# NoemieJaquier/GaBOtorch

Hardware: AMD Instinct MI355X
Metric: SPD affine-invariant kernel-matrix build, pairs/sec (N=4096,d=10) (higher is better)
Workload: dtype f64

## Files before the change

### gabotorch_amd/csrc/spd_pairwise_body.hpp

```cpp
#pragma once
#include "gabo_device.hpp"
#include "spd_eig.hpp"
#include "spd_prep.hpp"
#include "gabo_mirror.hpp"
#include "spd_generic.hpp"
#include "gabo_log_tab.hpp"
#include "gabo_exp_tab256.hpp"
#include "gabo_acosh2_table.hpp"
#include "../../include/gabo_hip.h"

#ifndef GABO_PAIR_WAVES
#define GABO_PAIR_WAVES 2
#else
#define GABO_PAIR_WAVES_FORCED 1
#endif

namespace gabo {

typedef const double __attribute__((address_space(1)))* spd_gcol_ptr;

struct SpdGcolBuffer {
    __amdgpu_buffer_rsrc_t rsrc;
    int voff;
    int stride_bytes;
    __device__ __forceinline__ double operator[](int k) const {
        return __builtin_bit_cast(double, __builtin_amdgcn_raw_buffer_load_b64(rsrc, voff, k * stride_bytes, 0));
    }
};
struct SpdGcolPointer {
    spd_gcol_ptr p;
    int64_t stride;
    __device__ __forceinline__ double operator[](int k) const { return p[(int64_t)k * stride]; }
};

template <int D, int WLIM>
struct SpdWGroups {
    int n = 0;
    int col[tri_size(D)] = {}, r0[tri_size(D)] = {}, r1[tri_size(D)] = {};
    constexpr SpdWGroups() {
        static_assert(WLIM >= D, "a row of the first column must fit a group");
        for (int c = D - 1; c >= 0; --c) {
            for (int r = c; r < D;) {
                int sum = 0;
                col[n] = c, r0[n] = r;
                while (r < D && sum + (r - c + 1) <= WLIM) sum += r - c + 1, ++r;
                r1[n++] = r;
            }
        }
    }
};
#ifndef GABO_PAIR_WLIM
#define GABO_PAIR_WLIM 16
#endif
template <int D, int AHEAD, class GCOL>
__device__ __forceinline__ void ai_congruence_staged(const double* __restrict__ W, const GCOL& Gj, double (&m)[tri_size(D)]) {
    constexpr SpdWGroups<D, (GABO_PAIR_WLIM < D ? D : GABO_PAIR_WLIM)> kG{};
    double gq[D][D];
    double wq[2][D][D];
    double c[D];
    auto issue_g = [&](auto ss) {
        constexpr int col = D - 1 - decltype(ss)::value;
        static_for<D - col>([&](auto kk) { gq[col][decltype(kk)::value] = Gj[tri(col + decltype(kk)::value, col)]; });
    };
    auto issue_w = [&](auto gg) {
        constexpr int g = decltype(gg)::value, col = kG.col[g], r0 = kG.r0[g], r1 = kG.r1[g];
        typedef const double __attribute__((address_space(4)))* wrow_ptr;
        wrow_ptr Wg = (wrow_ptr)W;
        asm volatile("" : "+s"(Wg));
        static_for<r1 - r0>([&](auto rr) {
            constexpr int r = r0 + decltype(rr)::value;
            static_for<r - col + 1>([&](auto kk) { wq[g & 1][r][col + decltype(kk)::value] = Wg[tri(r, col + decltype(kk)::value)]; });
        });
    };
    static_for<(AHEAD < D ? AHEAD : D)>(issue_g);
    issue_w(std::integral_constant<int, 0>{});
    static_for<kG.n>([&](auto gg) {
        constexpr int g = decltype(gg)::value, col = kG.col[g], r0 = kG.r0[g], r1 = kG.r1[g];
        if constexpr (r0 == col && D - 1 - col + AHEAD < D) issue_g(std::integral_constant<int, D - 1 - col + AHEAD>{});
        __builtin_amdgcn_sched_barrier(0);
        __builtin_amdgcn_s_waitcnt(0xc07f);
        __builtin_amdgcn_sched_barrier(0);
        if constexpr (g + 1 < kG.n) issue_w(std::integral_constant<int, g + 1>{});
        static_for<r1 - r0>([&](auto rr) {
            constexpr int r = r0 + decltype(rr)::value;
            double acc = wq[g & 1][r][col] * gq[col][0];
            static_for<r - col>([&](auto kk) {
                constexpr int k = col + 1 + decltype(kk)::value;
                acc = __builtin_fma(wq[g & 1][r][k], gq[col][k - col], acc);
            });
            c[r - col] = acc;
        });
        if constexpr (r1 == D) {
            __builtin_amdgcn_sched_barrier(0);
            static_for<D - col>([&](auto rr) {
                constexpr int r = col + decltype(rr)::value;
                static_for<r - col + 1>([&](auto qq) {
                    constexpr int q = col + decltype(qq)::value;
                    m[tri(r, q)] = col == q ? c[r - col] * c[q - col] : __builtin_fma(c[r - col], c[q - col], m[tri(r, q)]);
                });
            });
        }
    });
    __builtin_amdgcn_sched_barrier(0);
}

__constant__ double kLogTabRegs[8] = {1.41421356237309504880, 1.0 / 7.0, -1.0 / 6.0, 0.2, -0.25, 1.0 / 3.0, 6.93147180369123816490e-01,
                                      1.90821492927058770002e-10};
__device__ __forceinline__ LogTabRegs log_tab_regs_scalar() {
    typedef const double __attribute__((address_space(4)))* const_ptr;
    const_ptr p = (const_ptr)kLogTabRegs;
    asm volatile("" : "+s"(p));
    LogTabRegs t;
    t.sqrt2 = p[0], t.c7 = p[1], t.c6 = p[2], t.c5 = p[3], t.c4 = p[4], t.c3 = p[5], t.ln2_hi = p[6], t.ln2_lo = p[7];
    return t;
}

template <int D, int ORIENT = kQlOrientPerLane, int CTL = kQlCtlPlain, int AHEAD = 0, class GCOL>
__device__ __forceinline__ double ai_sumsq(const double* __restrict__ W, const GCOL& Gj, const double* __restrict__ ltab, const double eps2 = 0.0) {
    constexpr int T = tri_size(D);
    constexpr bool kDescending = ORIENT == kQlOrientLast;
    double m[T];
    if constexpr (AHEAD > 0) {
        static_assert(kDescending, "the staged congruence takes the columns from the last to the first");
        ai_congruence_staged<D, AHEAD>(W, Gj, m);
    } else
    static_for<D>([&](auto cc) {
        constexpr int col = kDescending ? D - 1 - decltype(cc)::value : decltype(cc)::value;
        double g[D - col], c[D - col];
        static_for<D - col>([&](auto kk) { g[decltype(kk)::value] = Gj[tri(col + decltype(kk)::value, col)]; });
        static_for<D - col>([&](auto rr) {
            constexpr int r = col + decltype(rr)::value;
            double acc = W[tri(r, col)] * g[0];
            static_for<r - col>([&](auto kk) {
                constexpr int k = col + 1 + decltype(kk)::value;
                acc = __builtin_fma(W[tri(r, k)], g[k - col], acc);
            });
            c[r - col] = acc;
        });
        static_for<D - col>([&](auto rr) {
            constexpr int r = col + decltype(rr)::value;
            static_for<r - col + 1>([&](auto qq) {
                constexpr int q = col + decltype(qq)::value;
                m[tri(r, q)] = (kDescending ? col == q : col == 0) ? c[r - col] * c[q - col] : __builtin_fma(c[r - col], c[q - col], m[tri(r, q)]);
            });
        });
    });
    double dg[D], e2[D];
    tridiagonalize<D, ORIENT>(m, dg, e2);
    tridiag_eigenvalues<D, ORIENT, CTL>(dg, e2, eps2);
    double s = 0.0;
    const LogTabRegs lr = AHEAD > 0 ? log_tab_regs_scalar() : LogTabRegs::load();
    static_for<D>([&](auto kk) { double lg = log_tab(dg[decltype(kk)::value], lr, ltab); s = __builtin_fma(lg, lg, s); });
    return s;
}

struct Spd2Col {
    double g00, g10, g11, lg;
};
__device__ __forceinline__ double ai_sumsq2(const double* __restrict__ W, const Spd2Col& g, double lw, const LogTabRegs& lr,
                                            const double* __restrict__ ltab, double tiny) {
    const double c00 = W[0] * g.g00, c11 = W[2] * g.g11;
    const double c10 = __builtin_fma(W[1], g.g00, W[2] * g.g10);
    const double m00 = c00 * c00, m10d = (c10 + c10) * c00, m11 = __builtin_fma(c10, c10, c11 * c11);
    const double tr = m00 + m11, df = m00 - m11;
    const double root = sqrt_nz(__builtin_fma(df, df, __builtin_fma(m10d, m10d, tiny)));
    const double l1 = log_tab(0.5 * (tr + root), lr, ltab);
    const double l2 = __builtin_fma(2.0, lw + g.lg, -l1);
    return __builtin_fma(l1, l1, l2 * l2);
}

__device__ __forceinline__ double finish(double dist, double beta, int mode) {
    if (mode == GABO_OUT_DISTANCE) return dist;
    if (mode == GABO_OUT_LAPLACE) return exp(-(dist * beta));
    return exp(-((dist * dist) * beta));
}

#ifndef GABO_PAIR_TWO_WAVE_MAX_DIM
#define GABO_PAIR_TWO_WAVE_MAX_DIM 14
#endif
#ifndef GABO_QL_EPS2_GAUSS
#define GABO_QL_EPS2_GAUSS 1e-14
#endif
constexpr bool spd_pair_gauss_only_instantiated(int d) { return d > 2 && d != 12; }
#ifndef GABO_PAIR_ORIENT
constexpr int spd_pair_gauss_only_orientation(int d) { return d == 14 ? kQlOrientCol0 : kQlOrientLast; }
#else
constexpr int spd_pair_gauss_only_orientation(int d) { return GABO_PAIR_ORIENT; }
#endif
#ifndef GABO_PAIR_SWEEPCTL
constexpr int spd_pair_gauss_only_sweepctl(int d) { return d == 20 ? kQlCtlPlain : (kQlCtlDenormalZero | kQlCtlHwSqrt | kQlCtlStageThreshold); }
#else
constexpr int spd_pair_gauss_only_sweepctl(int d) { return GABO_PAIR_SWEEPCTL; }
#endif
#ifndef GABO_PAIR_WAVES_FORCED
constexpr int spd_pair_gauss_only_waves(int d) { return d > GABO_PAIR_TWO_WAVE_MAX_DIM ? 1 : (d == 10 ? 3 : GABO_PAIR_WAVES); }
#else
constexpr int spd_pair_gauss_only_waves(int d) { return d > GABO_PAIR_TWO_WAVE_MAX_DIM ? 1 : GABO_PAIR_WAVES; }
#endif
#ifndef GABO_PAIR_AHEAD
constexpr int spd_pair_gauss_only_ahead(int d) { return d == 10 && spd_pair_gauss_only_waves(d) == 3 ? 2 : 0; }
#else
constexpr int spd_pair_gauss_only_ahead(int d) { return d == 10 ? GABO_PAIR_AHEAD : 0; }
#endif
template <int D, bool GAUSS_ONLY, bool BUFFER_ONLY>
__global__ __launch_bounds__(256, (GAUSS_ONLY ? spd_pair_gauss_only_waves(D) : (D > GABO_PAIR_TWO_WAVE_MAX_DIM ? 1 : GABO_PAIR_WAVES))) void spd_ai_pairwise_kernel(const double* __restrict__ Winv, const double* __restrict__ G,
                                                              double* __restrict__ out, double* __restrict__ dist_out_arg,
                                                              int64_t n1, int64_t n2,
                                                              int64_t w_batch_stride, int64_t g_batch_stride, int rows,
                                                              int col_blocks, int row_chunks, int64_t sym_tiles, double beta, int flags) {
    constexpr int T = tri_size(D);
    static_assert(GAUSS_ONLY == BUFFER_ONLY && (spd_pair_gauss_only_instantiated(D) || !GAUSS_ONLY), "instantiations that launch_spd_ai selects");
    const int mode = GAUSS_ONLY ? GABO_OUT_GAUSSIAN : (flags & GABO_OUT_MASK);
    double* const dist_out = GAUSS_ONLY ? nullptr : dist_out_arg;
    constexpr bool kTabExp = D <= 4;
    __shared__ double tab[kTabExp ? 64 : 1];
    __shared__ __attribute__((aligned(16))) double ltab[512];
    for (int k = threadIdx.x; k < 512; k += blockDim.x) ltab[k] = kLogTab[k];
    double ec[6], ec3 = 0.0;
    if constexpr (kTabExp) {
        if (threadIdx.x < 64) tab[threadIdx.x] = kExp2Tab[threadIdx.x];
    }
    __syncthreads();
    if constexpr (kTabExp) {
        static_for<6>([&](auto k) { ec[decltype(k)::value] = kExpTabC[decltype(k)::value]; });
        ec3 = ec[3];
        asm volatile("" : "+v"(ec3));
    }
    int64_t cg, rc, b;
    if (flags & GABO_SYMMETRIC) {
        const int64_t per_batch = sym_tiles;
        b = blockIdx.x / per_batch;
        int64_t t = blockIdx.x - b * per_batch;
        cg = 0;
        for (;;) {
            int64_t cnt = ((cg + 1) * (int64_t)blockDim.x + rows - 1) / rows;
            if (cnt > row_chunks) cnt = row_chunks;
            if (t < cnt) break;
            t -= cnt;
            ++cg;
        }
        rc = t;
    } else {
        const int64_t bid = blockIdx.x;
        cg = bid % col_blocks;
        rc = (bid / col_blocks) % row_chunks;
        b = bid / ((int64_t)col_blocks * row_chunks);
    }
    const int64_t j0 = cg * blockDim.x;
    const int64_t j = j0 + threadIdx.x;
    const int64_t jc = j < n2 ? j : n2 - 1;
    const int64_t i0 = rc * rows;
    const int64_t i1 = (i0 + rows < n1) ? i0 + rows : n1;
    if ((flags & GABO_SYMMETRIC) && j0 + (int64_t)(threadIdx.x | 63) < i0) return;
    const double* Gj = G + b * g_batch_stride + jc;
    double* ob = out + b * n1 * n2;
    const int64_t jw = j0 + (threadIdx.x & ~63);
    const bool use_buffer = BUFFER_ONLY || (D > 2 && (int64_t)T * n2 * 8 < (1ll << 31));
    SpdGcolBuffer gbuf;
    {
        const double* gw = G + b * g_batch_stride + (jw < n2 ? jw : n2 - 1);
        uint64_t a = (uint64_t)gw;
        a = ((uint64_t)(uint32_t)__builtin_amdgcn_readfirstlane((int)(a >> 32)) << 32) | (uint32_t)__builtin_amdgcn_readfirstlane((int)a);
        gbuf.rsrc = __builtin_amdgcn_make_buffer_rsrc((void*)a, 0, 0x7fffffff, 0x00020000);
        gbuf.voff = (int)((jc - (jw < n2 ? jw : n2 - 1)) * 8);
        gbuf.stride_bytes = (int)(n2 * 8);
    }
    Spd2Col col2;
    double lw_lane = 0.0, tiny = 1e-290;
    LogTabRegs lr2;
    if constexpr (D == 2) {
        lr2 = LogTabRegs::load();
        asm volatile("" : "+s"(tiny));
        col2.g00 = Gj[0];
        col2.g10 = Gj[n2];
        col2.g11 = Gj[2 * n2];
        col2.lg = log_tab(col2.g00 * col2.g11, lr2, ltab);
        int64_t ir = i0 + (threadIdx.x & 63);
        ir = ir < n1 ? ir : n1 - 1;
        const double* Wr = Winv + b * w_batch_stride + ir * T;
        lw_lane = log_tab(Wr[0] * Wr[2], lr2, ltab);
    }
    double eps2 = (mode == GABO_OUT_GAUSSIAN && !dist_out) ? GABO_QL_EPS2_GAUSS : 0.0;
    asm volatile("" : "+s"(eps2));
    if constexpr (GAUSS_ONLY && BUFFER_ONLY) {
        const int nrows = __builtin_amdgcn_readfirstlane((int)(i1 - i0));
        const int64_t jrel = j - i0;
        const int rmax = j >= n2 ? -1 : ((flags & GABO_SYMMETRIC) ? (jrel < 0 ? -1 : (jrel > rows - 1 ? rows - 1 : (int)jrel)) : rows - 1);
        const double* W = Winv + b * w_batch_stride + i0 * T;
        char* orow = reinterpret_cast<char*>(ob + i0 * n2 + j);
        for (int r = 0; r < nrows; ++r, W += T) {
            SpdGcolBuffer gb = gbuf;
            asm volatile("" : "+v"(gb.voff));
            asm volatile("" : "+s"(gb.stride_bytes));
            const double s = ai_sumsq<D, spd_pair_gauss_only_orientation(D), spd_pair_gauss_only_sweepctl(D), spd_pair_gauss_only_ahead(D)>(W, gb, ltab, eps2);
            double val;
            if constexpr (kTabExp) {
                val = exp_neg_tab(-((s + 1e-15) * beta), ec, ec3, tab);
                val = s != s ? s : val;
            } else {
                val = exp(-((s + 1e-15) * beta));
            }
            if (r <= rmax) *reinterpret_cast<double*>(orow) = val;
            orow += (unsigned)gb.stride_bytes;
        }
        return;
    }
    for (int64_t i = i0; i < i1; ++i) {
        const double* W = Winv + b * w_batch_stride + i * T;
        double s;
        if constexpr (D == 2) {
            const int lane = (int)(i - i0);
            const double lw = __hiloint2double(__builtin_amdgcn_readlane(__double2hiint(lw_lane), lane),
                                               __builtin_amdgcn_readlane(__double2loint(lw_lane), lane));
            s = ai_sumsq2(W, col2, lw, lr2, ltab, tiny);
        } else {
            if (use_buffer) {
                SpdGcolBuffer gb = gbuf;
                asm volatile("" : "+v"(gb.voff));
                asm volatile("" : "+s"(gb.stride_bytes));
                s = ai_sumsq<D>(W, gb, ltab, eps2);
            } else {
                SpdGcolPointer gp{(spd_gcol_ptr)Gj, n2};
                asm volatile("" : "+v"(gp.p));
                s = ai_sumsq<D>(W, gp, ltab, eps2);
            }
        }
        double dist, val;
        if (mode == GABO_OUT_GAUSSIAN && !dist_out) {
            dist = 0.0;
            if constexpr (kTabExp) {
                val = exp_neg_tab(-((s + 1e-15) * beta), ec, ec3, tab);
                val = s != s ? s : val;
            } else {
                val = exp(-((s + 1e-15) * beta));
            }
        } else {
            dist = __builtin_sqrt(s + 1e-15);
            val = finish(dist, beta, mode);
        }
        if (j < n2 && (!(flags & GABO_SYMMETRIC) || i <= j)) {
            ob[i * n2 + j] = val;
            if (dist_out) dist_out[b * n1 * n2 + i * n2 + j] = dist;
        }
    }
}

#ifndef GABO_GAUSS2_MAX_ROWS
#define GABO_GAUSS2_MAX_ROWS 64
#endif
constexpr double kGauss2L = 0.0027076061740622863;
__constant__ double kGauss2C[6] = {kGauss2L, kGauss2L * kGauss2L / 2.0, kGauss2L * kGauss2L * kGauss2L / 6.0,
                                   kGauss2L * kGauss2L * kGauss2L * kGauss2L / 24.0, 6755399441055744.0, 4096.0};

template <bool NT, bool SYM>
__global__ __launch_bounds__(256) void spd_ai_gauss2_kernel(const double* __restrict__ Winv, const double* __restrict__ G,
                                                            double* __restrict__ out, int64_t n1, int64_t n2, int64_t w_batch_stride,
                                                            int64_t g_batch_stride, int rows, int col_blocks, int row_chunks,
                                                            int64_t sym_tiles, double beta, int flags) {
    __shared__ __attribute__((aligned(16))) double ltab[512];
    __shared__ double etab[256];
    __shared__ __attribute__((aligned(16))) double atab[kAcosh2Slots * kAcosh2Stride];
    __shared__ __attribute__((aligned(16))) double wrow[GABO_GAUSS2_MAX_ROWS * 4];
    const int tid = threadIdx.x;
    for (int k = tid; k < 512; k += blockDim.x) ltab[k] = kLogTab[k];
    for (int k = tid; k < 256; k += blockDim.x) etab[k] = kExp2Tab256[k];
    {
        const double sc = beta * (-512.0 / 0.69314718055994530942), eps = beta * (-256.0 / 0.69314718055994530942) * 1e-15;
        constexpr int kUsedLo = (kAcosh2Binades - 1) * 16 * kAcosh2Stride, kUsedHi = 240 * kAcosh2Stride;
        for (int k = tid; k < kAcosh2Slots * kAcosh2Stride - (kUsedHi - kUsedLo); k += blockDim.x) {
            const int kk = k < kUsedLo ? k : k + (kUsedHi - kUsedLo);
            const double v = kAcosh2Tab[kk] * sc;
            atab[kk] = (kk % kAcosh2Stride == 0) ? v + eps : v;
        }
    }
    int64_t cg, rc, b;
    if constexpr (SYM) {
        const int64_t per_batch = sym_tiles;
        b = blockIdx.x / per_batch;
        int64_t t = blockIdx.x - b * per_batch;
        cg = 0;
        for (;;) {
            int64_t cnt = ((cg + 1) * (int64_t)blockDim.x + rows - 1) / rows;
            if (cnt > row_chunks) cnt = row_chunks;
            if (t < cnt) break;
            t -= cnt;
            ++cg;
        }
        rc = t;
    } else {
        const int64_t bid = blockIdx.x;
        cg = bid % col_blocks;
        rc = (bid / col_blocks) % row_chunks;
        b = bid / ((int64_t)col_blocks * row_chunks);
    }
    const int64_t j0 = cg * blockDim.x;
    const int64_t j = j0 + tid;
    const int64_t jc = j < n2 ? j : n2 - 1;
    const int64_t i0 = rc * rows;
    const int64_t i1 = (i0 + rows < n1) ? i0 + rows : n1;
    const double* Gj = G + b * g_batch_stride + jc;
    const double g00 = Gj[0], g10 = Gj[n2], g11 = Gj[2 * n2];
    const LogTabRegs lr = LogTabRegs::load();
    const double sscale = __builtin_sqrt(beta * (512.0 / 0.69314718055994530942));
    double w0l = 1.0, w1l = 0.0, w2l = 1.0;
    if (tid < rows) {
        int64_t ir = i0 + tid;
        ir = ir < n1 ? ir : n1 - 1;
        const double* Wr = Winv + b * w_batch_stride + ir * 3;
        w0l = Wr[0], w1l = Wr[1], w2l = Wr[2];
    }
    __syncthreads();
    if (tid < rows) {
        const double dw = w0l * w2l;
        const double sw = rsqrt_nz(dw + dw);
        wrow[4 * tid + 0] = w0l * sw;
        wrow[4 * tid + 1] = w1l * sw;
        wrow[4 * tid + 2] = w2l * sw;
        wrow[4 * tid + 3] = sscale * log_tab(dw, lr, ltab);
    }
    __syncthreads();
    if (SYM && j0 + (int64_t)(tid | 63) < i0) return;
    double ec[6];
    static_for<6>([&](auto k) { ec[decltype(k)::value] = kGauss2C[decltype(k)::value]; });
    double c4v = ec[3];
    asm volatile("" : "+v"(c4v));
    const double dg = g00 * g11;
    const double bcol = sscale * log_tab(dg, lr, ltab);
    const double sg = rsqrt_nz(dg);
    const double q00 = g00 * sg, q10 = g10 * sg, q11 = g11 * sg;
    double* orow = out + b * n1 * n2 + i0 * n2 + j;
    const int nrows = __builtin_amdgcn_readfirstlane((int)(i1 - i0));
    const int64_t jrel = j - i0;
    const int rmax = j >= n2 ? -1 : (SYM ? (jrel < 0 ? -1 : (jrel > GABO_GAUSS2_MAX_ROWS - 1 ? GABO_GAUSS2_MAX_ROWS - 1 : (int)jrel)) : GABO_GAUSS2_MAX_ROWS - 1);
    typedef double g2_v2d __attribute__((ext_vector_type(2)));
    if (!SYM && j >= n2) return;
    for (int r = 0; r < nrows; ++r, orow += n2) {
        const g2_v2d wa = *reinterpret_cast<const g2_v2d*>(wrow + 4 * r);
        const g2_v2d wb = *reinterpret_cast<const g2_v2d*>(wrow + 4 * r + 2);
        const double w0 = wa[0], w1 = wa[1], w2 = wb[0], arow = wb[1];
        const double hh = __builtin_fma(w0, q00, -(w2 * q11));
        const double cc = __builtin_fma(w1, q00, w2 * q10);
        const double tau = __builtin_fma(cc, cc, __builtin_fma(hh, hh, 1.0));
        const unsigned hi = (unsigned)__double2hiint(tau);
        static_assert(kAcosh2MBits == 4 && kAcosh2Slots == 256, "row index = 8 bits");
        const unsigned off = __umul24((hi >> 16) & 0xffu, (unsigned)(kAcosh2Stride * sizeof(double)));
        const double t = tau - __hiloint2double((int)(hi & ~((1u << (20 - kAcosh2MBits)) - 1u)), 0);
        const g2_v2d* row = reinterpret_cast<const g2_v2d*>(reinterpret_cast<const char*>(atab) + off);
        static_assert(kAcosh2Deg == 7, "four coefficient pairs");
        const g2_v2d c67 = row[3], c45 = row[2], c23 = row[1], c01 = row[0];
        double ya = __builtin_fma(c67[1], t, c67[0]);
        ya = __builtin_fma(ya, t, c45[1]);
        ya = __builtin_fma(ya, t, c45[0]);
        ya = __builtin_fma(ya, t, c23[1]);
        ya = __builtin_fma(ya, t, c23[0]);
        ya = __builtin_fma(ya, t, c01[1]);
        ya = __builtin_fma(ya, t, c01[0]);
        if (__builtin_expect(__any(!(tau < ec[5])), 0)) {
            if (!(tau < ec[5])) {
                const double dl = log(tau + __builtin_sqrt(__builtin_fma(tau, tau, -1.0)));
                ya = -(sscale * sscale) * __builtin_fma(dl, dl, 0.5e-15);
            }
        }
        const double sp = arow + bcol;
        const double y = __builtin_fma(-sp, sp, ya);
        const double km = y + ec[4];
        const double kk = km - ec[4];
        const double rr = y - kk;
        double p = __builtin_fma(rr, c4v, ec[2]);
        p = __builtin_fma(p, rr, ec[1]);
        p = __builtin_fma(p, rr, ec[0]);
        p = p * rr;
        const int ki = __double2loint(km);
        const double e = etab[ki & 255];
        const double val = __builtin_ldexp(__builtin_fma(e, p, e), ki >> 8);
        if (!SYM || r <= rmax) {
            if constexpr (NT) __builtin_nontemporal_store(val, orow);
            else *orow = val;
        }
    }
}

template <int D>
static int launch_spd_ai(const double* x1, const double* x2, double* out, double* dist_out, int64_t batch, int64_t n1, int64_t n2,
                         int64_t s1, int64_t s2, double beta, int flags, double* ws, int* status, hipStream_t st, bool prepared = false) {
    constexpr int T = tri_size(D);
    const int64_t b1 = (s1 == 0) ? 1 : batch;
    const int64_t b2 = (s2 == 0) ? 1 : batch;
    double* W = ws;
    double* G = ws + b1 * n1 * T;
    if (!prepared) launch_spd_prep<D>(x1, x2, W, G, b1, b2, n1, n2, s1, s2, status, st, 1);
#ifndef GABO_PAIR_THREADS
#define GABO_PAIR_THREADS (D >= 7 ? 64 : 256)
#endif
    int threads = n2 >= 256 ? GABO_PAIR_THREADS : (n2 > 128 ? 192 : (n2 > 64 ? 128 : 64));
    int64_t col_blocks = (n2 + threads - 1) / threads;
#ifndef GABO_PAIR_ROWS_D2
#define GABO_PAIR_ROWS_D2 16
#endif
#ifndef GABO_PAIR_ROWS
#define GABO_PAIR_ROWS (D >= 9 ? 8 : 16)
#endif
#ifndef GABO_PAIR_ROWS_GAUSS2
#define GABO_PAIR_ROWS_GAUSS2 64
#endif
    const bool gauss2 = D == 2 && (flags & GABO_OUT_MASK) == GABO_OUT_GAUSSIAN && !dist_out && beta >= 0.0;
    int rows = D == 2 ? (gauss2 ? GABO_PAIR_ROWS_GAUSS2 : GABO_PAIR_ROWS_D2) : GABO_PAIR_ROWS;
    while (rows > 1 && col_blocks * ((n1 + rows - 1) / rows) * batch < (rows > 16 ? 1024 : 4096)) rows >>= 1;
    int64_t row_chunks = (n1 + rows - 1) / rows;
    int64_t sym_tiles = 0;
    if (flags & GABO_SYMMETRIC) {
        for (int64_t cg = 0; cg < col_blocks; ++cg) {
            int64_t cnt = ((cg + 1) * threads + rows - 1) / rows;
            sym_tiles += cnt < row_chunks ? cnt : row_chunks;
        }
    }
    int64_t nblocks = ((flags & GABO_SYMMETRIC) ? sym_tiles : col_blocks * row_chunks) * batch;
    if (nblocks > 0x7fffffffLL) return GABO_ERR_ARG;
    bool special2 = false;
    if constexpr (D == 2) special2 = gauss2 && rows <= GABO_GAUSS2_MAX_ROWS;
    if (special2) {
        const bool streaming = batch * n1 * n2 * 8 > (32ll << 20) && !(flags & GABO_SYMMETRIC);
#define GABO_GAUSS2_LAUNCH(...)                                                                                                     \
        hipLaunchKernelGGL((spd_ai_gauss2_kernel<__VA_ARGS__>), dim3((unsigned)nblocks), dim3(threads), 0, st, W, G, out, n1, n2,           \
                           (s1 == 0) ? (int64_t)0 : n1 * T, (s2 == 0) ? (int64_t)0 : n2 * T, rows, (int)col_blocks, (int)row_chunks,       \
                           sym_tiles, beta, flags)
        if (flags & GABO_SYMMETRIC) GABO_GAUSS2_LAUNCH(false, true);
        else if (streaming) GABO_GAUSS2_LAUNCH(true, false);
        else GABO_GAUSS2_LAUNCH(false, false);
#undef GABO_GAUSS2_LAUNCH
    } else {
#define GABO_PAIR_LAUNCH(...)                                                                                                             \
        hipLaunchKernelGGL((spd_ai_pairwise_kernel<D, __VA_ARGS__>), dim3((unsigned)nblocks), dim3(threads), 0, st, W, G, out, dist_out, n1, n2, \
                           (s1 == 0) ? (int64_t)0 : n1 * T, (s2 == 0) ? (int64_t)0 : n2 * T, rows, (int)col_blocks, (int)row_chunks,       \
                           sym_tiles, beta, flags)
        bool gauss_only = false;
        if constexpr (spd_pair_gauss_only_instantiated(D)) {
            gauss_only = (flags & GABO_OUT_MASK) == GABO_OUT_GAUSSIAN && !dist_out && (int64_t)T * n2 * 8 < (1ll << 31);
            if (gauss_only) GABO_PAIR_LAUNCH(true, true);
        }
        if (!gauss_only) GABO_PAIR_LAUNCH(false, false);
#undef GABO_PAIR_LAUNCH
    }
    if (flags & GABO_SYMMETRIC) {
        int tiles = (int)((n1 + 31) / 32);
        hipLaunchKernelGGL((mirror_upper_kernel<0>), dim3((unsigned)((int64_t)tiles * (tiles + 1) / 2), (unsigned)batch), dim3(256), 0, st,
                           out, n1, tiles);
        if (dist_out)
            hipLaunchKernelGGL((mirror_upper_kernel<0>), dim3((unsigned)((int64_t)tiles * (tiles + 1) / 2), (unsigned)batch), dim3(256), 0,
                               st, dist_out, n1, tiles);
    }
    return hipGetLastError() == hipSuccess ? GABO_OK : GABO_ERR_LAUNCH;
}

}

namespace gabo {
int launch_spd_ai_prepared(int d, double* out, int64_t batch, int64_t n1, int64_t n2, bool shared1, bool shared2, double beta, int flags,
                           double* ws, hipStream_t st);
int launch_spd_ai_wide2(int d, const double* x1, const double* x2, double* out, double* dist_out, int64_t batch, int64_t n1, int64_t n2,
                        int64_t s1, int64_t s2, double beta, int flags, double* ws, int* status, hipStream_t st);
int launch_spd_ai_wide3(int d, const double* x1, const double* x2, double* out, double* dist_out, int64_t batch, int64_t n1, int64_t n2,
                        int64_t s1, int64_t s2, double beta, int flags, double* ws, int* status, hipStream_t st);
int launch_spd_ai_wide(int d, const double* x1, const double* x2, double* out, double* dist_out, int64_t batch, int64_t n1, int64_t n2,
                       int64_t s1, int64_t s2, double beta, int flags, double* ws, int* status, hipStream_t st);
}
```

Before: 8.126 billion.

## Store mirrored lower triangle in Gaussian kernel and decode symmetric tiles in closed form

For symmetric Gaussian-only launches, each thread parks its computed row values in LDS and then writes the transposed entries itself. This removes the separate mirror_upper kernel launch and its extra pass over the output matrix. Block-to-tile decoding for symmetric grids also swaps the linear search loop for a closed-form sqrt-based triangular inverse, and 32-bit uniform decode is used elsewhere. In exchange the kernel takes dynamic LDS, which may reduce occupancy, and the transposed stores are strided, column-wise and poorly coalesced.

```diff
diff --git a/gabotorch_amd/csrc/gabo_sym_tiles.hpp b/gabotorch_amd/csrc/gabo_sym_tiles.hpp
--- /dev/null
+++ b/gabotorch_amd/csrc/gabo_sym_tiles.hpp
@@ -0,0 +1,55 @@
+#pragma once
+#include <cstdint>
+
+#if !defined(__HIPCC__) && !defined(__host__)
+#define __host__
+#define __device__
+#endif
+
+namespace gabo {
+
+__host__ __device__ inline int64_t sym_tile_count(int64_t col_blocks, int threads, int rows, int64_t row_chunks) {
+    int64_t tiles = 0;
+    for (int64_t cg = 0; cg < col_blocks; ++cg) {
+        const int64_t cnt = ((cg + 1) * threads + rows - 1) / rows;
+        tiles += cnt < row_chunks ? cnt : row_chunks;
+    }
+    return tiles;
+}
+
+__host__ __device__ inline uint32_t sym_tri_prefix(uint32_t c, uint32_t q) {
+    return q * ((c & 1u) ? c * ((c + 1u) >> 1) : (c >> 1) * (c + 1u));
+}
+
+__host__ __device__ inline uint32_t sym_tri_group(uint32_t t, uint32_t q, uint32_t guess) {
+    uint32_t c = guess;
+    if (sym_tri_prefix(c, q) > t) --c;
+    if (sym_tri_prefix(c + 1u, q) <= t) ++c;
+    return c;
+}
+
+__host__ __device__ inline uint32_t sym_tri_guess(uint32_t t, uint32_t q) {
+    return (uint32_t)(int32_t)(__builtin_sqrtf(2.0f * (float)t / (float)q + 0.25f) - 0.5f);
+}
+
+struct SymTile {
+    uint32_t cg, rc;
+};
+
+__host__ __device__ inline SymTile sym_tile_from_guess(uint32_t t, uint32_t q, uint32_t row_chunks, uint32_t guess) {
+    const uint32_t c = sym_tri_group(t, q, guess);
+    if ((c + 1u) * q < row_chunks) return {c, t - sym_tri_prefix(c, q)};
+    const uint32_t cap = (row_chunks + q - 1u) / q - 1u;
+    const uint32_t u = t - sym_tri_prefix(cap, q);
+    const uint32_t k = u / row_chunks;
+    return {cap + k, u - k * row_chunks};
+}
+
+__host__ __device__ inline uint32_t sym_tile_q(uint32_t threads, uint32_t rows) { return threads >> __builtin_ctz(rows); }
+
+__host__ __device__ inline SymTile sym_tile_of(uint32_t t, uint32_t threads, uint32_t rows, uint32_t row_chunks) {
+    const uint32_t q = sym_tile_q(threads, rows);
+    return sym_tile_from_guess(t, q, row_chunks, sym_tri_guess(t, q));
+}
+
+}
diff --git a/gabotorch_amd/csrc/spd_pairwise_body.hpp b/gabotorch_amd/csrc/spd_pairwise_body.hpp
--- a/gabotorch_amd/csrc/spd_pairwise_body.hpp
+++ b/gabotorch_amd/csrc/spd_pairwise_body.hpp
@@ -3,6 +3,7 @@
 #include "spd_eig.hpp"
 #include "spd_prep.hpp"
 #include "gabo_mirror.hpp"
+#include "gabo_sym_tiles.hpp"
 #include "spd_generic.hpp"
 #include "gabo_log_tab.hpp"
 #include "gabo_exp_tab256.hpp"
@@ -202,7 +203,58 @@
 #else
 constexpr int spd_pair_gauss_only_ahead(int d) { return d == 10 ? GABO_PAIR_AHEAD : 0; }
 #endif
-template <int D, bool GAUSS_ONLY, bool BUFFER_ONLY>
+#ifndef GABO_PAIR_SYM_DECODE
+#define GABO_PAIR_SYM_DECODE 1
+#endif
+constexpr bool spd_pair_closed_form_decode() { return GABO_PAIR_SYM_DECODE != 0; }
+#ifndef GABO_PAIR_SYM_MIRROR
+#define GABO_PAIR_SYM_MIRROR 1
+#endif
+constexpr bool spd_pair_gauss_only_stores_mirror(int d) {
+    return GABO_PAIR_SYM_MIRROR != 0 && spd_pair_gauss_only_instantiated(d) && d <= 11 && d != 7;
+}
+#ifndef GABO_PAIR_ROWS
+#define GABO_PAIR_ROWS (D >= 9 ? 8 : 16)
+#endif
+
+__device__ __forceinline__ void spd_pair_block_tile(bool sym, int rows, int col_blocks, int row_chunks, int64_t sym_tiles, int64_t& cg,
+                                                    int64_t& rc, int64_t& b) {
+    auto uni = [](uint32_t v) { return (int64_t)(uint32_t)__builtin_amdgcn_readfirstlane((int)v); };
+    if (sym) {
+        if constexpr (spd_pair_closed_form_decode()) {
+            const uint32_t per_batch = (uint32_t)sym_tiles, bb = blockIdx.x / per_batch;
+            const uint32_t t = blockIdx.x - bb * per_batch, q = sym_tile_q(blockDim.x, (uint32_t)rows);
+            const SymTile tile = sym_tile_from_guess(t, q, (uint32_t)row_chunks, (uint32_t)__builtin_amdgcn_readfirstlane((int)sym_tri_guess(t, q)));
+            cg = uni(tile.cg), rc = uni(tile.rc), b = uni(bb);
+        } else {
+            const int64_t per_batch = sym_tiles;
+            b = blockIdx.x / per_batch;
+            int64_t t = blockIdx.x - b * per_batch;
+            cg = 0;
+            for (;;) {
+                int64_t cnt = ((cg + 1) * (int64_t)blockDim.x + rows - 1) / rows;
+                if (cnt > row_chunks) cnt = row_chunks;
+                if (t < cnt) break;
+                t -= cnt;
+                ++cg;
+            }
+            rc = t;
+        }
+    } else if constexpr (spd_pair_closed_form_decode()) {
+        const uint32_t bid = blockIdx.x, row = bid / (uint32_t)col_blocks;
+        const uint32_t bb = row / (uint32_t)row_chunks;
+        cg = uni(bid - row * (uint32_t)col_blocks), rc = uni(row - bb * (uint32_t)row_chunks), b = uni(bb);
+    } else {
+        const int64_t bid = blockIdx.x;
+        cg = bid % col_blocks;
+        rc = (bid / col_blocks) % row_chunks;
+        b = bid / ((int64_t)col_blocks * row_chunks);
+    }
+}
+
+template <int D>
+constexpr int kSpdPairParkStride = GABO_PAIR_ROWS + 3;
+template <int D, bool GAUSS_ONLY, bool BUFFER_ONLY, bool MIRROR = false>
 __global__ __launch_bounds__(256, (GAUSS_ONLY ? spd_pair_gauss_only_waves(D) : (D > GABO_PAIR_TWO_WAVE_MAX_DIM ? 1 : GABO_PAIR_WAVES))) void spd_ai_pairwise_kernel(const double* __restrict__ Winv, const double* __restrict__ G,
                                                               double* __restrict__ out, double* __restrict__ dist_out_arg,
                                                               int64_t n1, int64_t n2,
@@ -210,6 +262,7 @@
                                                               int col_blocks, int row_chunks, int64_t sym_tiles, double beta, int flags) {
     constexpr int T = tri_size(D);
     static_assert(GAUSS_ONLY == BUFFER_ONLY && (spd_pair_gauss_only_instantiated(D) || !GAUSS_ONLY), "instantiations that launch_spd_ai selects");
+    static_assert(!MIRROR || (GAUSS_ONLY && spd_pair_gauss_only_stores_mirror(D)), "the lower triangle is stored by Gaussian-only x1-is-x2 launches alone");
     const int mode = GAUSS_ONLY ? GABO_OUT_GAUSSIAN : (flags & GABO_OUT_MASK);
     double* const dist_out = GAUSS_ONLY ? nullptr : dist_out_arg;
     constexpr bool kTabExp = D <= 4;
@@ -227,31 +280,14 @@
         asm volatile("" : "+v"(ec3));
     }
     int64_t cg, rc, b;
-    if (flags & GABO_SYMMETRIC) {
-        const int64_t per_batch = sym_tiles;
-        b = blockIdx.x / per_batch;
-        int64_t t = blockIdx.x - b * per_batch;
-        cg = 0;
-        for (;;) {
-            int64_t cnt = ((cg + 1) * (int64_t)blockDim.x + rows - 1) / rows;
-            if (cnt > row_chunks) cnt = row_chunks;
-            if (t < cnt) break;
-            t -= cnt;
-            ++cg;
-        }
-        rc = t;
-    } else {
-        const int64_t bid = blockIdx.x;
-        cg = bid % col_blocks;
-        rc = (bid / col_blocks) % row_chunks;
-        b = bid / ((int64_t)col_blocks * row_chunks);
-    }
+    const bool sym = MIRROR || (flags & GABO_SYMMETRIC);
+    spd_pair_block_tile(sym, rows, col_blocks, row_chunks, sym_tiles, cg, rc, b);
     const int64_t j0 = cg * blockDim.x;
     const int64_t j = j0 + threadIdx.x;
     const int64_t jc = j < n2 ? j : n2 - 1;
     const int64_t i0 = rc * rows;
     const int64_t i1 = (i0 + rows < n1) ? i0 + rows : n1;
-    if ((flags & GABO_SYMMETRIC) && j0 + (int64_t)(threadIdx.x | 63) < i0) return;
+    if (sym && j0 + (int64_t)(threadIdx.x | 63) < i0) return;
     const double* Gj = G + b * g_batch_stride + jc;
     double* ob = out + b * n1 * n2;
     const int64_t jw = j0 + (threadIdx.x & ~63);
@@ -285,9 +321,16 @@
     if constexpr (GAUSS_ONLY && BUFFER_ONLY) {
         const int nrows = __builtin_amdgcn_readfirstlane((int)(i1 - i0));
         const int64_t jrel = j - i0;
-        const int rmax = j >= n2 ? -1 : ((flags & GABO_SYMMETRIC) ? (jrel < 0 ? -1 : (jrel > rows - 1 ? rows - 1 : (int)jrel)) : rows - 1);
+        const int rmax = j >= n2 ? -1 : (sym ? (jrel < 0 ? -1 : (jrel > rows - 1 ? rows - 1 : (int)jrel)) : rows - 1);
         const double* W = Winv + b * w_batch_stride + i0 * T;
         char* orow = reinterpret_cast<char*>(ob + i0 * n2 + j);
+        extern __shared__ double park_lds[];
+        double* const park = park_lds + threadIdx.x * kSpdPairParkStride<D>;
+        if constexpr (MIRROR) {
+            park[GABO_PAIR_ROWS] = __builtin_bit_cast(double, ob + j * n2 + i0);
+            park[GABO_PAIR_ROWS + 1] = __hiloint2double(0, jrel > rows - 1 ? rmax : rmax - 1);
+            asm volatile("" ::: "memory");
+        }
         for (int r = 0; r < nrows; ++r, W += T) {
             SpdGcolBuffer gb = gbuf;
             asm volatile("" : "+v"(gb.voff));
@@ -302,6 +345,14 @@
             }
             if (r <= rmax) *reinterpret_cast<double*>(orow) = val;
             orow += (unsigned)gb.stride_bytes;
+            if constexpr (MIRROR) park[r] = val;
+        }
+        if constexpr (MIRROR) {
+            typedef double __attribute__((address_space(1)))* gout_ptr;
+            const gout_ptr mrow = (gout_ptr)__builtin_bit_cast(double*, park[GABO_PAIR_ROWS]);
+            const int mmax = __double2loint(park[GABO_PAIR_ROWS + 1]);
+            for (int r = 0; r < nrows; ++r)
+                if (r <= mmax) mrow[r] = park[r];
         }
         return;
     }
@@ -374,25 +425,7 @@
         }
     }
     int64_t cg, rc, b;
-    if constexpr (SYM) {
-        const int64_t per_batch = sym_tiles;
-        b = blockIdx.x / per_batch;
-        int64_t t = blockIdx.x - b * per_batch;
-        cg = 0;
-        for (;;) {
-            int64_t cnt = ((cg + 1) * (int64_t)blockDim.x + rows - 1) / rows;
-            if (cnt > row_chunks) cnt = row_chunks;
-            if (t < cnt) break;
-            t -= cnt;
-            ++cg;
-        }
-        rc = t;
-    } else {
-        const int64_t bid = blockIdx.x;
-        cg = bid % col_blocks;
-        rc = (bid / col_blocks) % row_chunks;
-        b = bid / ((int64_t)col_blocks * row_chunks);
-    }
+    spd_pair_block_tile(SYM, rows, col_blocks, row_chunks, sym_tiles, cg, rc, b);
     const int64_t j0 = cg * blockDim.x;
     const int64_t j = j0 + tid;
     const int64_t jc = j < n2 ? j : n2 - 1;
@@ -497,9 +530,6 @@
 #ifndef GABO_PAIR_ROWS_D2
 #define GABO_PAIR_ROWS_D2 16
 #endif
-#ifndef GABO_PAIR_ROWS
-#define GABO_PAIR_ROWS (D >= 9 ? 8 : 16)
-#endif
 #ifndef GABO_PAIR_ROWS_GAUSS2
 #define GABO_PAIR_ROWS_GAUSS2 64
 #endif
@@ -507,16 +537,10 @@
     int rows = D == 2 ? (gauss2 ? GABO_PAIR_ROWS_GAUSS2 : GABO_PAIR_ROWS_D2) : GABO_PAIR_ROWS;
     while (rows > 1 && col_blocks * ((n1 + rows - 1) / rows) * batch < (rows > 16 ? 1024 : 4096)) rows >>= 1;
     int64_t row_chunks = (n1 + rows - 1) / rows;
-    int64_t sym_tiles = 0;
-    if (flags & GABO_SYMMETRIC) {
-        for (int64_t cg = 0; cg < col_blocks; ++cg) {
-            int64_t cnt = ((cg + 1) * threads + rows - 1) / rows;
-            sym_tiles += cnt < row_chunks ? cnt : row_chunks;
-        }
-    }
+    const int64_t sym_tiles = (flags & GABO_SYMMETRIC) ? sym_tile_count(col_blocks, threads, rows, row_chunks) : 0;
     int64_t nblocks = ((flags & GABO_SYMMETRIC) ? sym_tiles : col_blocks * row_chunks) * batch;
     if (nblocks > 0x7fffffffLL) return GABO_ERR_ARG;
-    bool special2 = false;
+    bool special2 = false, mirrored = false;
     if constexpr (D == 2) special2 = gauss2 && rows <= GABO_GAUSS2_MAX_ROWS;
     if (special2) {
         const bool streaming = batch * n1 * n2 * 8 > (32ll << 20) && !(flags & GABO_SYMMETRIC);
@@ -529,22 +553,27 @@
         else GABO_GAUSS2_LAUNCH(false, false);
 #undef GABO_GAUSS2_LAUNCH
     } else {
-#define GABO_PAIR_LAUNCH(...)                                                                                                             \
-        hipLaunchKernelGGL((spd_ai_pairwise_kernel<D, __VA_ARGS__>), dim3((unsigned)nblocks), dim3(threads), 0, st, W, G, out, dist_out, n1, n2, \
+#define GABO_PAIR_LAUNCH(LDS_BYTES, ...)                                                                                                  \
+        hipLaunchKernelGGL((spd_ai_pairwise_kernel<D, __VA_ARGS__>), dim3((unsigned)nblocks), dim3(threads), LDS_BYTES, st, W, G, out, dist_out, n1, n2, \
                            (s1 == 0) ? (int64_t)0 : n1 * T, (s2 == 0) ? (int64_t)0 : n2 * T, rows, (int)col_blocks, (int)row_chunks,       \
                            sym_tiles, beta, flags)
         bool gauss_only = false;
         if constexpr (spd_pair_gauss_only_instantiated(D)) {
             gauss_only = (flags & GABO_OUT_MASK) == GABO_OUT_GAUSSIAN && !dist_out && (int64_t)T * n2 * 8 < (1ll << 31);
-            if (gauss_only) GABO_PAIR_LAUNCH(true, true);
-        }
-        if (!gauss_only) GABO_PAIR_LAUNCH(false, false);
+            if constexpr (spd_pair_gauss_only_stores_mirror(D)) {
+                mirrored = gauss_only && (flags & GABO_SYMMETRIC);
+                if (mirrored) GABO_PAIR_LAUNCH(threads * kSpdPairParkStride<D> * sizeof(double), true, true, true);
+            }
+            if (gauss_only && !mirrored) GABO_PAIR_LAUNCH(0, true, true);
+        }
+        if (!gauss_only) GABO_PAIR_LAUNCH(0, false, false);
 #undef GABO_PAIR_LAUNCH
     }
     if (flags & GABO_SYMMETRIC) {
         int tiles = (int)((n1 + 31) / 32);
-        hipLaunchKernelGGL((mirror_upper_kernel<0>), dim3((unsigned)((int64_t)tiles * (tiles + 1) / 2), (unsigned)batch), dim3(256), 0, st,
-                           out, n1, tiles);
+        if (!mirrored)
+            hipLaunchKernelGGL((mirror_upper_kernel<0>), dim3((unsigned)((int64_t)tiles * (tiles + 1) / 2), (unsigned)batch), dim3(256), 0, st,
+                               out, n1, tiles);
         if (dist_out)
             hipLaunchKernelGGL((mirror_upper_kernel<0>), dim3((unsigned)((int64_t)tiles * (tiles + 1) / 2), (unsigned)batch), dim3(256), 0,
                                st, dist_out, n1, tiles);
```

Result: no change. 8.133 billion, median of 4 (+0.1%).
